# TAMUCrypto/virgo-plus

Hardware: AMD Instinct MI355X
Metric: prover sec + field-ops/sec, SHA-256 circuit, 1/2/4/8 MI355X (bit-exact) (higher is better)
Workload: dtype u64 (F_p^2, p=2^61-1); 1 GPU; SHA-256 1024-block circuit (SHA256_64.pws x1024, 102347776 gates, 15 layers, 2^23 input wires), GKR sumcheck + Virgo FFT/LDT commit on GPU (BASELINE configs[2]); pass_mode=sync, field_ops_per_proof=8299342697

## Files before the change

### virgo-plus_amd/__init__.py

```python
import ctypes
import os
import shutil
import subprocess

PKG_DIR = os.path.dirname(os.path.abspath(__file__))
ROOT = os.path.dirname(PKG_DIR)
CSRC = os.path.join(PKG_DIR, "csrc")
HOST = os.path.join(PKG_DIR, "host")
LIB_GPU = os.environ.get("VP_LIBGPU") or os.path.join(CSRC, "libvpgpu.so")
LIB_GPU_CHECKED = os.path.join(ROOT, "tools", "_build", "checked", "libvpgpu.so")
LIB_GPU_TESTDRV = os.path.join(ROOT, "tools", "_build", "testdrv", "libvpgpu.so")
LIB_HOST = os.path.join(HOST, "libvphost.so")
CLI = os.path.join(HOST, "virgo_plus_run")

GPU_SRC = [os.path.join(CSRC, f) for f in ("vpgpu.hip", "vpgpu_batched.inc", "vpgpu_pc.inc", "vpgpu_pc_shard.inc", "vpgpu_fftgkr.inc", "vpgpu_upload.inc", "vp_kernels_fftgkr.h", "vp_kernels.h", "vp_kernels_round.h", "vp_kernels_persist.h", "vp_kernels_batch.h",
                                              "vp_kernels_plan.h", "vp_kernels_pc.h", "vp_kernels_ntt8.h", "vp_kernels_ntt_long.h", "vp_keccak_asm.h", "vp_check.h", "vp_field.h")] + [
    os.path.join(ROOT, "include", "vpgpu.h")]
HOST_SRC = [os.path.join(HOST, f) for f in ("circuit.cpp", "prover.cpp", "verifier.cpp", "vphost.cpp")]
HOST_HDR = [os.path.join(HOST, f) for f in ("circuit.hpp", "prover.hpp", "verifier.hpp", "vphost.h", "field.hpp",
                                              "polynomial.hpp")]


def _stale(target, sources):
    if not os.path.exists(target):
        return True
    t = os.path.getmtime(target)
    return any(os.path.getmtime(s) > t for s in sources if os.path.exists(s))


def _hipcc():
    for c in (shutil.which("hipcc"), "/opt/rocm/bin/hipcc"):
        if c and os.path.exists(c):
            return c
    return None


def build(force=False, verbose=False):
    def run(cmd):
        if verbose:
            print(" ".join(cmd), flush=True)
        subprocess.run(cmd, check=True)

    if os.environ.get("VP_LIBGPU"):
        pass
    elif force or _stale(LIB_GPU, GPU_SRC):
        hipcc = _hipcc()
        if hipcc is None:
            if os.path.exists(LIB_GPU):
                return
# ... 951 lines not shown
```

### virgo-plus_amd/csrc/vp_field.h

```cpp
#pragma once
#include <stdint.h>

#if defined(__HIPCC__)
#define VP_HD __host__ __device__ __forceinline__
#else
#define VP_HD inline
#endif

namespace vp {

typedef unsigned long long u64;
typedef unsigned int u32;
typedef unsigned __int128 u128;

constexpr u64 P61 = 2305843009213693951ull;

struct alignas(16) F {
    u64 re, im;
};

VP_HD F f_make(u64 re, u64 im) { F r; r.re = re; r.im = im; return r; }
VP_HD F f_zero() { return f_make(0, 0); }
VP_HD F f_one() { return f_make(1, 0); }
VP_HD bool f_eq(const F &a, const F &b) { return a.re == b.re && a.im == b.im; }
// ... 110 lines not shown
}
template <bool WEAK = false, bool MS = false>
VP_HD F f_mad31_rb(const F &a, u64 y, const F &c) {
    const Sp31 ar = split31(a.re), ai = split31(a.im), b = split31(y);
    return f_make(dot1_31<WEAK, MS>(ar, b, c.re), dot1_31<WEAK, MS>(ai, b, c.im));
}
template <bool WEAK, bool MS = false>
VP_HD F f_mad31c_rb(const F &a, u64 y, const F &c) {
    const Sp31 ar = split31(a.re), ai = split31(a.im), b = split31(y);
    return f_make(dot1_31c<WEAK, MS>(ar, b, c.re), dot1_31c<WEAK, MS>(ai, b, c.im));
}
template <bool MS = false>
VP_HD u64 dot4_31cc(const Sp31 &x0, const Sp31 &y0, const Sp31 &x1, const Sp31 &y1, const Sp31 &x2, const Sp31 &y2, const Sp31 &x3, const Sp31 &y3) {
    const u64 L = (u64) x0.lo * y0.lo + (u64) x1.lo * y1.lo + (u64) x2.lo * y2.lo + (u64) x3.lo * y3.lo;
    const u64 C = (u64) x0.lo * y0.hi + (u64) x0.hi * y0.lo + (u64) x1.lo * y1.hi + (u64) x1.hi * y1.lo
                + (u64) x2.lo * y2.hi + (u64) x2.hi * y2.lo + (u64) x3.lo * y3.hi + (u64) x3.hi * y3.lo;
    const u64 H = (u64) x0.hi * y0.hi + (u64) x1.hi * y1.hi + (u64) x2.hi * y2.hi + (u64) x3.hi * y3.hi;
    u64 s = c31_add<MS>(C, (L & P61) + (L >> 61)) + (H << 1);
    s = (s & P61) + (s >> 61);
    return s >= P61 ? s - P61 : s;
}
template <bool MS = false>
VP_HD F f_dot2cc(const F &a, const F &b, const F &c, const F &d) {
#if defined(__HIP_DEVICE_COMPILE__) && !defined(VP_MUL128)
    const Sp31 ar = split31(a.re), ai = split31(a.im), nai = split31(P61 - a.im), br = split31(b.re), bi = split31(b.im);
    const Sp31 cr = split31(c.re), ci = split31(c.im), nci = split31(P61 - c.im), dr = split31(d.re), di = split31(d.im);
    return f_make(dot4_31cc<MS>(ar, br, nai, bi, cr, dr, nci, di), dot4_31cc<MS>(ar, bi, ai, br, cr, di, ci, dr));
#else
    return f_add(f_mul128(a, b), f_mul128(c, d));
#endif
}
VP_HD F f_lerp(const F &a, const F &b, const F &r) { return f_add(a, f_mul(r, f_sub(b, a))); }

}
```

### virgo-plus_amd/csrc/vp_kernels_batch.h

```cpp
#pragma once
#include "vp_kernels_round.h"

namespace vp {

struct Half { const F *bf; const F *bs; int h1; int pad; };
__device__ __forceinline__ F half_at(const Half &h, u32 i) {
    return f_mul(h.bf[i & ((1u << h.h1) - 1)], h.bs[i >> h.h1]);
}
__device__ __forceinline__ F half_mad(const Half &h, u32 i, const F &c) {
    return f_mad31c<false, VP_MADSHIFT != 0>(h.bf[i & ((1u << h.h1) - 1)], h.bs[i >> h.h1], c);
}

struct InitArgs2 {
    const u32 *rowptr; const u32 *e_g; const u32 *e_x; const uint16_t *e_tl;
    Half hg, hu;
    F *const *vals;
    const F *gc;
    const F *Vu;
    const F *assert_r;
    F *V, *M, *A;
    const uint8_t *s_layer; const u32 *s_idx;
    u32 n_rows;
    int vreal;
    const unsigned long long *const *valsr;
};
__device__ __forceinline__ F mul_val(const InitArgs2 &a, const F &y, const F &t) {
    return a.vreal ? f_mad31c_rb<false>(t, y.re, f_zero()) : f_mul(y, t);
}
__device__ __forceinline__ F val_at(const InitArgs2 &a, int l, u32 x) {
    return (a.vreal && a.valsr) ? f_make(a.valsr[l][x], 0) : a.vals[l][x];
}

template <int PHASE>
__device__ __forceinline__ void contrib2(const InitArgs2 &a, u32 e, F &m, F &ad, const F &vu) {
    const u32 g = a.e_g[e], x = a.e_x[e], tl = a.e_tl[e];
    const int ty = (tl >> 8) & 0x7f;
    F t = half_at(a.hg, g);
    if (tl & 0x8000) t = f_mul(t, *a.assert_r);
    if (PHASE == 1) {
        const int l = tl & 0xff;
        F ty_ = f_zero();
        if (l != 0xff && VP_CHK_LAYER(l, x)) ty_ = mul_val(a, val_at(a, l, x), t);
        switch (ty) {
            case T_ADD: ad = f_add(ad, ty_); m = f_add(m, t); break;
            case T_SUB: ad = f_sub(ad, ty_); m = f_add(m, t); break;
            case T_ANTISUB: ad = f_add(ad, ty_); m = f_sub(m, t); break;
            case T_MUL: m = f_add(m, ty_); break;
            case T_NAAB: ad = f_add(ad, ty_); m = f_sub(m, ty_); break;
            case T_ANTINAAB: m = f_add(m, f_sub(t, ty_)); break;
            case T_ADDC: ad = f_add(ad, f_mul(a.gc[g], t)); m = f_add(m, t); break;
            case T_MULC: m = f_add(m, f_mul(a.gc[g], t)); break;
            case T_COPY: m = f_add(m, t); break;
            case T_NOT: ad = f_add(ad, t); m = f_sub(m, t); break;
            case T_XOR: ad = f_add(ad, ty_); m = f_add(m, f_sub(t, f_dbl(ty_))); break;
            default: break;
        }
    } else {
        t = f_mul(t, half_at(a.hu, x));
        const F tv = f_mul(t, vu);
        switch (ty) {
            case T_ADD: m = f_add(m, t); ad = f_add(ad, tv); break;
            case T_SUB: m = f_sub(m, t); ad = f_add(ad, tv); break;
            case T_ANTISUB: m = f_add(m, t); ad = f_sub(ad, tv); break;
            case T_MUL: m = f_add(m, tv); break;
            case T_NAAB: m = f_add(m, f_sub(t, tv)); break;
            case T_ANTINAAB: m = f_sub(m, tv); ad = f_add(ad, tv); break;
            case T_XOR: ad = f_add(ad, tv); m = f_add(m, f_sub(t, f_dbl(tv))); break;
            case T_COPY: ad = f_add(ad, tv); break;
            case T_NOT: ad = f_add(ad, f_sub(t, tv)); break;
            case T_ADDC: ad = f_add(ad, f_mul(t, f_add(a.gc[g], vu))); break;
            case T_MULC: ad = f_add(ad, f_mul(tv, a.gc[g])); break;
            default: break;
        }
    }
}

struct P1Entry { u32 g, x, tl; };
struct P1Vals { F bf, bs, y; };
__device__ __forceinline__ P1Entry p1_load(const InitArgs2 &a, u32 e) { P1Entry c; c.g = a.e_g[e]; c.x = a.e_x[e]; c.tl = a.e_tl[e]; return c; }
__device__ __forceinline__ P1Vals p1_gather(const InitArgs2 &a, const P1Entry &c) {
    P1Vals v;
    v.bf = a.hg.bf[c.g & ((1u << a.hg.h1) - 1)]; v.bs = a.hg.bs[c.g >> a.hg.h1];
    const int l = c.tl & 0xff;
    v.y = (l != 0xff && VP_CHK_LAYER(l, c.x)) ? val_at(a, l, c.x) : f_zero();
    return v;
}
__device__ __forceinline__ void p1_apply(const InitArgs2 &a, const P1Entry &c, const P1Vals &v, F &m, F &ad) {
    const int ty = (c.tl >> 8) & 0x7f;
    F t = f_mul(v.bf, v.bs);
    if (c.tl & 0x8000) t = f_mul(t, *a.assert_r);
    F ty_ = f_zero();
    if ((c.tl & 0xff) != 0xff) ty_ = mul_val(a, v.y, t);
    switch (ty) {
        case T_ADD: ad = f_add(ad, ty_); m = f_add(m, t); break;
        case T_SUB: ad = f_sub(ad, ty_); m = f_add(m, t); break;
        case T_ANTISUB: ad = f_add(ad, ty_); m = f_sub(m, t); break;
        case T_MUL: m = f_add(m, ty_); break;
        case T_NAAB: ad = f_add(ad, ty_); m = f_sub(m, ty_); break;
        case T_ANTINAAB: m = f_add(m, f_sub(t, ty_)); break;
        case T_ADDC: ad = f_add(ad, f_mul(a.gc[c.g], t)); m = f_add(m, t); break;
        case T_MULC: m = f_add(m, f_mul(a.gc[c.g], t)); break;
        case T_COPY: m = f_add(m, t); break;
        case T_NOT: ad = f_add(ad, t); m = f_sub(m, t); break;
        case T_XOR: ad = f_add(ad, ty_); m = f_add(m, f_sub(t, f_dbl(ty_))); break;
        default: break;
    }
}

template <int PHASE>
__device__ __forceinline__ void init2_light_body(const InitArgs2 &a, u32 bid) {
    u32 row = bid * blockDim.x + threadIdx.x;
    if (row >= a.n_rows) return;
    if (PHASE == 2) {
        const int l = a.s_layer[row];
        if (l != 0xfe) a.V[row] = (l == 0xff || !VP_CHK((unsigned) l < g_vp_chk_layers() && a.s_idx[row] < g_vp_chk_lsize(l), 2, l, a.s_idx[row], row)) ? f_zero() : val_at(a, l, a.s_idx[row]);
    }
    u32 b = a.rowptr[row], e = a.rowptr[row + 1];
    if (!VP_CHK(b <= e, 3, row, b, e)) return;
    if (e - b > VP_LIGHT_MAX) return;
    F m = f_zero(), ad = f_zero();
    const F vu = PHASE == 2 ? *a.Vu : f_zero();
    for (u32 k = b; k < e; ++k) contrib2<PHASE>(a, k, m, ad, vu);
    a.M[row] = m;
    a.A[row] = ad;
}
template <int PHASE>
__global__ void __launch_bounds__(VP_BLOCK) k_init2_light(InitArgs2 a) { init2_light_body<PHASE>(a, blockIdx.x); }

struct ChunkFuse { const u32 *chunk_h; const u32 *heavy_row; const u32 *heavy_cptr; u32 *heavy_cnt; F *M; F *A; };
template <int PHASE>
__device__ __forceinline__ void init2_chunks_body(const InitArgs2 &a, const u32 *__restrict__ chunk_beg, const u32 *__restrict__ chunk_end,
                                                  u32 n_chunks, F *__restrict__ part, u32 bid, const ChunkFuse *fuse = nullptr) {
    const u32 c = bid * (blockDim.x >> 6) + (threadIdx.x >> 6);
    if (c >= n_chunks) return;
    const int lane = threadIdx.x & 63;
    F m = f_zero(), ad = f_zero();
    const F vu = PHASE == 2 ? *a.Vu : f_zero();
    for (u32 k = chunk_beg[c] + lane; k < chunk_end[c]; k += 64) contrib2<PHASE>(a, k, m, ad, vu);
    m = wave_sum(m);
    ad = wave_sum(ad);
    if (!fuse) { if (lane == 0) { part[2 * c] = m; part[2 * c + 1] = ad; } return; }
    const u32 h = fuse->chunk_h[c], c0 = fuse->heavy_cptr[h], n = fuse->heavy_cptr[h + 1] - c0, row = fuse->heavy_row[h];
    if (n == 1) { if (lane == 0) { fuse->M[row] = m; fuse->A[row] = ad; } return; }
    int last = 0;
    if (lane == 0) {
        unsigned long long *w = reinterpret_cast<unsigned long long *>(part + 2 * c);
        cf_st(w, m.re); cf_st(w + 1, m.im); cf_st(w + 2, ad.re); cf_st(w + 3, ad.im);
        asm volatile("s_waitcnt vmcnt(0)" ::: "memory");
        last = __hip_atomic_fetch_add(fuse->heavy_cnt + h, 1u, __ATOMIC_RELAXED, __HIP_MEMORY_SCOPE_AGENT) == n - 1;
    }
    last = __builtin_amdgcn_readfirstlane(last);
    if (!last) return;
    F tm = f_zero(), ta = f_zero();
    for (u32 i = lane; i < n; i += 64) {
        const unsigned long long *w = reinterpret_cast<const unsigned long long *>(part + 2 * (c0 + i));
        tm = f_add(tm, f_make(cf_ld(w), cf_ld(w + 1))); ta = f_add(ta, f_make(cf_ld(w + 2), cf_ld(w + 3)));
    }
    tm = wave_sum(tm); ta = wave_sum(ta);
    if (lane == 0) { fuse->M[row] = tm; fuse->A[row] = ta; __hip_atomic_store(fuse->heavy_cnt + h, 0u, __ATOMIC_RELAXED, __HIP_MEMORY_SCOPE_AGENT); }
}
template <int PHASE>
__global__ void __launch_bounds__(VP_BLOCK)
k_init2_chunks(InitArgs2 a, const u32 *__restrict__ chunk_beg, const u32 *__restrict__ chunk_end, u32 n_chunks,
               F *__restrict__ part) { init2_chunks_body<PHASE>(a, chunk_beg, chunk_end, n_chunks, part, blockIdx.x); }

__device__ __forceinline__ void liu_gather_body(const u32 *__restrict__ rowptr, const uint8_t *__restrict__ e_q, const u32 *__restrict__ e_g,
                                                const Half *__restrict__ H, u32 size, F *__restrict__ M, u32 bid, u32 u0 = 0) {
    u32 u = bid * blockDim.x + threadIdx.x;
    if (u >= size) return;
    F m = half_at(H[0], u0 + u);
    if (!VP_CHK(rowptr[u] <= rowptr[u + 1], 4, u, rowptr[u], rowptr[u + 1])) return;
    for (u32 k = rowptr[u]; k < rowptr[u + 1]; ++k) if (VP_CHK(e_q[k] < g_vp_chk_liu(), 4, u, k, e_q[k])) m = f_add(m, half_at(H[e_q[k]], e_g[k]));
    M[u] = m;
// ... 45 lines not shown
    const F dv = f_sub_lazy(v1, v0), dm = f_sub_lazy(m1, m0);
    lz_add(X, f_mad_lazy<true>(dm, dv, f_zero()));
    if (keep_y) lz_add(Y, f_mad_c<true>(m1, v1, HAS_A ? a1 : f_zero()));
    lz_add(Z, f_mad_c<true>(m0, v0, HAS_A ? a0 : f_zero()));
    vo = sf_fold<false>(r, dv, v0);
    mo = sf_fold<false>(r, dm, m0);
    if (HAS_A) ao = sf_fold<false>(r, f_sub_lazy(a1, a0), a0);
}

template <bool HAS_A>
__device__ __forceinline__ void sf_pair_step_rv(u64 v0, u64 v1, const F &m0, const F &m1, const F &a0, const F &a1,
                                                const F &r, Lz &X, Lz &Y, Lz &Z, F &vo, F &mo, F &ao, bool keep_y) {
    const u64 dv = v1 + P61 - v0;
    const F dm = f_sub_lazy(m1, m0);
    lz_add(X, f_mad31_rb<true, VP_MADSHIFT>(dm, dv, f_zero()));
    if (keep_y) lz_add(Y, f_mad31c_rb<true, VP_MADSHIFT>(m1, v1, HAS_A ? a1 : f_zero()));
    lz_add(Z, f_mad31c_rb<true, VP_MADSHIFT>(m0, v0, HAS_A ? a0 : f_zero()));
    vo = f_mad31c_rb<false, VP_MADSHIFT>(r, dv, f_make(v0, 0));
    mo = sf_fold<false>(r, dm, m0);
    if (HAS_A) ao = sf_fold<false>(r, f_sub_lazy(a1, a0), a0);
}

struct Sf3bLds { F s1[3][256]; F s2[3][128]; F red[4][9]; Lz acc2[3][128]; Lz acc3[3][64]; F dred[4]; };

struct GenLoad { static constexpr int MODE = 0; };
struct GenP1 {
    static constexpr int MODE = 1;
    const InitArgs2 *a; Half dot_h; F *dot_part;
    __device__ __forceinline__ void row(u32 row, u32 valid, F &m, F &ad) const {
        m = f_zero(); ad = f_zero();
        if (row >= valid || row >= a->n_rows) return;
        const u32 b = a->rowptr[row], e = a->rowptr[row + 1];
        if (e - b > VP_LIGHT_MAX) { m = a->M[row]; ad = a->A[row]; return; }
        for (u32 k = b; k < e; ++k) contrib2<1>(*a, k, m, ad, f_zero());
    }
    __device__ __forceinline__ void ptrs(u32 r0, u32 valid, u32 &b0, u32 &e0, u32 &e1) const {
        const u32 lim = min(valid, a->n_rows);
        b0 = e0 = e1 = 0;
        if (r0 >= lim) return;
        b0 = a->rowptr[r0]; e0 = a->rowptr[r0 + 1];
        e1 = r0 + 1 < lim ? a->rowptr[r0 + 2] : e0;
    }
    __device__ __forceinline__ void row2(u32 r0, u32 valid, u32 b0, u32 e0, u32 e1, F &m0, F &a0, F &m1, F &a1) const {
        m0 = f_zero(); a0 = f_zero(); m1 = f_zero(); a1 = f_zero();
        const u32 lim = min(valid, a->n_rows);
        if (r0 >= lim) return;
        const bool heavy0 = e0 - b0 > VP_LIGHT_MAX, heavy1 = e1 - e0 > VP_LIGHT_MAX;
        const bool f0 = !heavy0 && e0 > b0, f1 = !heavy1 && e1 > e0;
        P1Entry c0{}, c1{};
        if (f0) c0 = p1_load(*a, b0);
        if (f1) c1 = p1_load(*a, e0);
        P1Vals v0{}, v1{};
        if (f0) v0 = p1_gather(*a, c0);
        if (f1) v1 = p1_gather(*a, c1);
        if (heavy0) { m0 = a->M[r0]; a0 = a->A[r0]; }
        if (heavy1) { m1 = a->M[r0 + 1]; a1 = a->A[r0 + 1]; }
        if (f0) p1_apply(*a, c0, v0, m0, a0);
        if (f1) p1_apply(*a, c1, v1, m1, a1);
        if (!heavy0) for (u32 k = b0 + 1; k < e0; ++k) contrib2<1>(*a, k, m0, a0, f_zero());
        if (!heavy1) for (u32 k = e0 + 1; k < e1; ++k) contrib2<1>(*a, k, m1, a1, f_zero());
    }
};
struct GenLiu {
    static constexpr int MODE = 2;
    const u32 *rowptr; const uint8_t *e_q; const u32 *e_g; const Half *H;
    __device__ __forceinline__ void row(u32 u, u32 valid, F &m, F &ad) const {
        ad = f_zero(); m = f_zero();
        if (u >= valid) return;
        m = half_at(H[0], u);
        for (u32 k = rowptr[u]; k < rowptr[u + 1]; ++k) m = f_add(m, half_at(H[e_q[k]], e_g[k]));
    }
    __device__ __forceinline__ void ptrs(u32 u0, u32 valid, u32 &b0, u32 &e0, u32 &e1) const {
        b0 = e0 = e1 = 0;
        if (u0 >= valid) return;
        b0 = rowptr[u0]; e0 = rowptr[u0 + 1];
        e1 = u0 + 1 < valid ? rowptr[u0 + 2] : e0;
    }
    __device__ __forceinline__ void row2(u32 u0, u32 valid, u32 b0, u32 e0, u32 e1, F &m0, F &a0, F &m1, F &a1) const {
        m0 = f_zero(); a0 = f_zero(); m1 = f_zero(); a1 = f_zero();
        if (u0 >= valid) return;
        const bool ok1 = u0 + 1 < valid;
        const Half h0 = H[0];
        const F bf0 = h0.bf[u0 & ((1u << h0.h1) - 1)], bs0 = h0.bs[u0 >> h0.h1];
        F bf1 = f_zero(), bs1 = f_zero();
        if (ok1) { bf1 = h0.bf[(u0 + 1) & ((1u << h0.h1) - 1)]; bs1 = h0.bs[(u0 + 1) >> h0.h1]; }
        const bool f0 = e0 > b0, f1 = e1 > e0;
        u32 q0 = 0, g0 = 0, q1 = 0, g1 = 0;
        if (f0) { q0 = e_q[b0]; g0 = e_g[b0]; }
        if (f1) { q1 = e_q[e0]; g1 = e_g[e0]; }
        Half hq0 = h0, hq1 = h0;
        if (f0) hq0 = H[q0];
        if (f1) hq1 = H[q1];
        F xf0 = f_zero(), xs0 = f_zero(), xf1 = f_zero(), xs1 = f_zero();
        if (f0) { xf0 = hq0.bf[g0 & ((1u << hq0.h1) - 1)]; xs0 = hq0.bs[g0 >> hq0.h1]; }
        if (f1) { xf1 = hq1.bf[g1 & ((1u << hq1.h1) - 1)]; xs1 = hq1.bs[g1 >> hq1.h1]; }
        m0 = f_dot2cc<VP_MADSHIFT != 0>(bf0, bs0, xf0, xs0);
        if (ok1) m1 = f_dot2cc<VP_MADSHIFT != 0>(bf1, bs1, xf1, xs1);
        for (u32 k = b0 + 1; k < e0; ++k) m0 = half_mad(H[e_q[k]], e_g[k], m0);
        for (u32 k = e0 + 1; k < e1; ++k) m1 = half_mad(H[e_q[k]], e_g[k], m1);
    }
};

struct GenP2 {
    static constexpr int MODE = 3;
    const InitArgs2 *a;
    __device__ __forceinline__ F vrow(u32 row, u32 vend) const {
        if (row >= vend || row >= a->n_rows) return f_zero();
        const int l = a->s_layer[row];
        if (l == 0xff || l == 0xfe) return f_zero();
        const u32 x = a->s_idx[row];
        if (!VP_CHK((unsigned) l < g_vp_chk_layers() && x < g_vp_chk_lsize(l), 2, l, x, row)) return f_zero();
        return val_at(*a, l, x);
    }
    __device__ __forceinline__ void ptrs(u32 r0, u32 valid, u32 &b0, u32 &e0, u32 &e1) const {
        const u32 lim = min(valid, a->n_rows);
        b0 = e0 = e1 = 0;
        if (r0 >= lim) return;
        b0 = a->rowptr[r0]; e0 = a->rowptr[r0 + 1];
        e1 = r0 + 1 < lim ? a->rowptr[r0 + 2] : e0;
    }
    __device__ __forceinline__ void row2(u32 r0, u32 valid, u32 b0, u32 e0, u32 e1, F &m0, F &a0, F &m1, F &a1) const {
        m0 = f_zero(); a0 = f_zero(); m1 = f_zero(); a1 = f_zero();
        const u32 lim = min(valid, a->n_rows);
        if (r0 >= lim) return;
        const bool heavy0 = e0 - b0 > VP_LIGHT_MAX, heavy1 = e1 - e0 > VP_LIGHT_MAX;
        if (heavy0) { m0 = a->M[r0]; a0 = a->A[r0]; }
        if (heavy1) { m1 = a->M[r0 + 1]; a1 = a->A[r0 + 1]; }
        const F vu = *a->Vu;
        u32 k0 = heavy0 ? e0 : b0, k1 = heavy1 ? e1 : e0;
        while (k0 < e0 && k1 < e1) { contrib2<2>(*a, k0++, m0, a0, vu); contrib2<2>(*a, k1++, m1, a1, vu); }
        for (; k0 < e0; ++k0) contrib2<2>(*a, k0, m0, a0, vu);
        for (; k1 < e1; ++k1) contrib2<2>(*a, k1, m1, a1, vu);
    }
};

template <bool HAS_A, class Gen>
__device__ __forceinline__ void sumfold3b_body(const SfArgs &a, u32 bid, u32 nb, Sf3bLds &sm, const Gen &gen) {
    F (&s1)[3][256] = sm.s1; F (&s2)[3][128] = sm.s2; F (&red)[4][9] = sm.red;
    const int t = threadIdx.x, lane = t & 63, w = t >> 6;
    Lz acc[3];
#pragma unroll
    for (int i = 0; i < 3; ++i) acc[i].re = acc[i].im = 0;
    if (t < 128) { for (int i = 0; i < 3; ++i) { sm.acc2[i][t].re = 0; sm.acc2[i][t].im = 0; } }
    if (t < 64) { for (int i = 0; i < 3; ++i) { sm.acc3[i][t].re = 0; sm.acc3[i][t].im = 0; } }
    const F r0 = a.r[0], r1 = a.r[1], r2 = a.r[2];
    const bool keep_y0 = (a.keep_y0 & 1) != 0, keep_rest = (a.keep_y0 & 2) != 0;
    const bool vreal = (a.keep_y0 & 4) != 0;
    F dacc = f_zero();
    for (u32 c = bid; c < a.total_chunks; c += nb) {
        int j = 0;
        while (j + 1 < a.n_tab && c >= a.t[j + 1].chunk_start) ++j;
        const SfTab td = a.t[j];
        const u32 cl = c - td.chunk_start;
        const int wl = w, tl = t;
        const u32 i0 = td.off + cl * 512 + 2 * tl, vend = td.off + td.valid;
        {
            F v0, v1, m0, m1, a0 = f_zero(), a1 = f_zero();
            if constexpr (Gen::MODE == 3) { v0 = gen.vrow(i0, vend); v1 = gen.vrow(i0 + 1, vend); }
            else if (vreal && a.inVr) {
                v0 = f_make(i0 < vend ? a.inVr[i0] : 0ull, 0); v1 = f_make(i0 + 1 < vend ? a.inVr[i0 + 1] : 0ull, 0);
            } else {
                if (cl * 512 + 512 <= td.valid) { v0 = a.inV[i0]; v1 = a.inV[i0 + 1]; }
                else { v0 = ld_or_zero(a.inV, i0, vend); v1 = ld_or_zero(a.inV, i0 + 1, vend); }
            }
            if constexpr (Gen::MODE == 0) {
// ... 102 lines not shown
```

### virgo-plus_amd/csrc/vp_kernels_plan.h

```cpp
#pragma once
#include "vp_kernels_batch.h"

namespace vp {

#ifndef VP_SEG_LOG
#define VP_SEG_LOG 10
#endif
#define VP_SEG (1 << VP_SEG_LOG)
#define VP_SEG_THREADS 768

struct SegTab {
    u32 off;
    u32 valid;
    u32 seg_start;
    int seg_log;
};
struct SegArgs {
    const F *inV, *inM, *inA;
    F *outV, *outM, *outA;
    const F *r;
    F *part;
    u32 part_stride;
    u32 total_segs;
    int n_tab, n_rounds;
// ... 457 lines not shown
__global__ void __launch_bounds__(VP_BLOCK) k_dotfin_multi(const DotJob *__restrict__ jobs) {
    __shared__ F lds[4];
    const DotJob &j = jobs[blockIdx.x];
    F acc[1] = {f_zero()};
    for (u32 i = threadIdx.x; i < j.nblk; i += blockDim.x) acc[0] = f_add(acc[0], j.part[i]);
    block_sum<1>(acc, lds);
    if (threadIdx.x == 0) *j.out = acc[0];
}
__global__ void k_vu_place(const F *__restrict__ sums, F *const *__restrict__ dst, u32 n) {
    const u32 c = blockIdx.x * blockDim.x + threadIdx.x;
    if (c >= n) return;
    F v = sums[c];
    v.re = m_red128((u128) v.re); v.im = m_red128((u128) v.im);
    *dst[c] = v;
}
__global__ void __launch_bounds__(VP_BLOCK) k_chunks_multi(const ChunkJob *__restrict__ jobs, const BlkMap *__restrict__ map) {
    const BlkMap m = map[blockIdx.x];
    const ChunkJob &j = jobs[m.job];
    if (j.phase == 1) init2_chunks_body<1>(j.a, j.chunk_beg, j.chunk_end, j.n_chunks, j.part, m.bid, j.fused ? &j.fuse : nullptr);
    else init2_chunks_body<2>(j.a, j.chunk_beg, j.chunk_end, j.n_chunks, j.part, m.bid, j.fused ? &j.fuse : nullptr);
}
__global__ void __launch_bounds__(VP_BLOCK) k_combine_multi(const CombineJob *__restrict__ jobs, const BlkMap *__restrict__ map) {
    const BlkMap m = map[blockIdx.x];
    const CombineJob &j = jobs[m.job];
    init_combine_body(j.heavy_row, j.heavy_cptr, j.n_heavy, j.part, j.M, j.A, m.bid);
}
__global__ void __launch_bounds__(VP_BLOCK, VP_SF_MINB) k_sumfold3b_multi(const SfArgs *__restrict__ jobs, const BlkMap *__restrict__ map) {
    __shared__ Sf3bLds sm;
    const BlkMap m = map[blockIdx.x];
    const SfArgs &a = jobs[m.job];
    if (a.has_a) sumfold3b_body<true>(a, m.bid, a.nblk, sm, GenLoad()); else sumfold3b_body<false>(a, m.bid, a.nblk, sm, GenLoad());
}
struct SfGenJob { SfArgs sf; InitArgs2 a; GatherJob g; Half dot_h; F *dot_part; int mode; int pad; };
__global__ void __launch_bounds__(VP_BLOCK, VP_SF_MINB) k_sumfold3b_gen_multi(const SfGenJob *__restrict__ jobs, const BlkMap *__restrict__ map) {
    __shared__ Sf3bLds sm;
    const BlkMap m = map[blockIdx.x];
    const SfGenJob &j = jobs[m.job];
    if (j.mode == 1) {
        GenP1 g; g.a = &j.a; g.dot_h = j.dot_h; g.dot_part = j.dot_part;
        sumfold3b_body<true>(j.sf, m.bid, j.sf.nblk, sm, g);
    } else if (j.mode == 3) {
        GenP2 g; g.a = &j.a;
        sumfold3b_body<true>(j.sf, m.bid, j.sf.nblk, sm, g);
    } else {
        GenLiu g; g.rowptr = j.g.rowptr; g.e_q = j.g.e_q; g.e_g = j.g.e_g; g.H = j.g.H;
        sumfold3b_body<false>(j.sf, m.bid, j.sf.nblk, sm, g);
    }
}
__global__ void __launch_bounds__(VP_SEG_THREADS) k_seg_multi(const SegArgs *__restrict__ jobs, const BlkMap *__restrict__ map) {
    __shared__ SegLds sm;
    const BlkMap m = map[blockIdx.x];
    const SegArgs &a = jobs[m.job];
    if (a.has_a) seg_body<true>(a, m.bid, a.nblk, sm); else seg_body<false>(a, m.bid, a.nblk, sm);
}
__global__ void __launch_bounds__(VP_EMIT_THREADS) k_emit_multi(const EmitArgs *__restrict__ jobs) {
    extern __shared__ __align__(16) unsigned char smem_raw[];
    emit_body(jobs[blockIdx.x], smem_raw);
}

}
```

### virgo-plus_amd/csrc/vp_kernels_round.h

```cpp
#pragma once
#include <hip/hip_runtime.h>
#include "vp_field.h"

namespace vp {

#define VP_MAX_TAB 64
#define VP_BLOCK 256
#define VP_LIGHT_MAX 16
#define VP_CHUNK 512

enum { T_MUL = 0, T_ADD, T_SUB, T_ANTISUB, T_NAAB, T_ANTINAAB, T_INPUT, T_MULC, T_ADDC, T_XOR, T_NOT, T_COPY };

__device__ __forceinline__ F ldF(const F *p) { return *p; }

template <int CTRL, int ROW_MASK>
__device__ __forceinline__ u64 dpp_u64(u64 v) {
    const u32 lo = __builtin_amdgcn_update_dpp(0u, (u32) v, CTRL, ROW_MASK, 0xf, false);
    const u32 hi = __builtin_amdgcn_update_dpp(0u, (u32) (v >> 32), CTRL, ROW_MASK, 0xf, false);
    return ((u64) hi << 32) | lo;
}
__device__ __forceinline__ u64 m_fold(u64 s) {
    s = (s & P61) + (s >> 61);
    return s >= P61 ? s - P61 : s;
}
__device__ __forceinline__ F wave_sum63(F x) {
    u64 a = x.re, b = x.im;
    a += dpp_u64<0x111, 0xf>(a); b += dpp_u64<0x111, 0xf>(b);
    a += dpp_u64<0x112, 0xf>(a); b += dpp_u64<0x112, 0xf>(b);
    a += dpp_u64<0x114, 0xf>(a); b += dpp_u64<0x114, 0xf>(b);
    a = m_fold(a); b = m_fold(b);
    a += dpp_u64<0x118, 0xf>(a); b += dpp_u64<0x118, 0xf>(b);
    a += dpp_u64<0x142, 0xa>(a); b += dpp_u64<0x142, 0xa>(b);
    a += dpp_u64<0x143, 0xc>(a); b += dpp_u64<0x143, 0xc>(b);
    return f_make(m_fold(a), m_fold(b));
}
__device__ __forceinline__ F wave_sum(F x) {
    const F t = wave_sum63(x);
    F r;
    r.re = ((u64) __builtin_amdgcn_readlane((u32) (t.re >> 32), 63) << 32) | (u32) __builtin_amdgcn_readlane((u32) t.re, 63);
    r.im = ((u64) __builtin_amdgcn_readlane((u32) (t.im >> 32), 63) << 32) | (u32) __builtin_amdgcn_readlane((u32) t.im, 63);
    return r;
}

template <int N>
__device__ __forceinline__ void block_sum(F (&x)[N], F *lds ) {
    const int lane = threadIdx.x & 63, w = threadIdx.x >> 6;
#pragma unroll
    for (int i = 0; i < N; ++i) x[i] = wave_sum(x[i]);
    if (lane == 0) {
#pragma unroll
        for (int i = 0; i < N; ++i) lds[w * N + i] = x[i];
    }
    __syncthreads();
    if (threadIdx.x == 0) {
        const int nw = blockDim.x >> 6;
#pragma unroll
// ... 123 lines not shown
__global__ void __launch_bounds__(VP_BLOCK)
k_beta_expand(const F *__restrict__ bf, const F *__restrict__ bs, int h1, u32 count, F *__restrict__ out) {
    const u32 mask = (1u << h1) - 1;
    for (u32 i = blockIdx.x * blockDim.x + threadIdx.x; i < count; i += gridDim.x * blockDim.x)
        out[i] = f_mul(bf[i & mask], bs[i >> h1]);
}

__global__ void k_scale_entries(F *beta, const u32 *__restrict__ idx, u32 n, const F *__restrict__ s) {
    u32 i = blockIdx.x * blockDim.x + threadIdx.x;
    if (i < n) beta[idx[i]] = f_mul(beta[idx[i]], *s);
}

struct InitArgs {
    const u32 *rowptr;
    const u32 *e_g;
    const u32 *e_x;
    const uint16_t *e_tl;
    const F *beta_g;
    const F *beta_u;
    F *const *vals;
    const F *gc;
    const F *coef;
    F *M, *A;
    u32 n_rows;
};

template <int PHASE>
__device__ __forceinline__ void contrib(const InitArgs &a, u32 e, F &m, F &ad) {
    const u32 g = a.e_g[e];
    const u32 x = a.e_x[e];
    const u32 tl = a.e_tl[e];
    const int ty = (tl >> 8) & 0x7f;
    if (PHASE == 1) {
        const F t = a.beta_g[g];
        const int l = tl & 0xff;
        F ty_ = f_zero();
        if (l != 0xff) ty_ = f_mul(a.vals[l][x], t);
        switch (ty) {
            case T_ADD: ad = f_add(ad, ty_); m = f_add(m, t); break;
            case T_SUB: ad = f_sub(ad, ty_); m = f_add(m, t); break;
            case T_ANTISUB: ad = f_add(ad, ty_); m = f_sub(m, t); break;
            case T_MUL: m = f_add(m, ty_); break;
            case T_NAAB: ad = f_add(ad, ty_); m = f_sub(m, ty_); break;
            case T_ANTINAAB: m = f_add(m, f_sub(t, ty_)); break;
            case T_ADDC: ad = f_add(ad, f_mul(a.gc[g], t)); m = f_add(m, t); break;
            case T_MULC: m = f_add(m, f_mul(a.gc[g], t)); break;
            case T_COPY: m = f_add(m, t); break;
            case T_NOT: ad = f_add(ad, t); m = f_sub(m, t); break;
            case T_XOR: ad = f_add(ad, ty_); m = f_add(m, f_sub(t, f_dbl(ty_))); break;
            default: break;
        }
    } else {
        const F t = f_mul(a.beta_g[g], a.beta_u[x]);
        F cm = a.coef[2 * ty], ca = a.coef[2 * ty + 1];
        if (ty == T_ADDC) ca = f_add(a.gc[g], ca);
        if (ty == T_MULC) ca = f_mul(a.gc[g], ca);
        m = f_add(m, f_mul(t, cm));
        ad = f_add(ad, f_mul(t, ca));
    }
}

template <int PHASE>
__global__ void __launch_bounds__(VP_BLOCK) k_init_light(InitArgs a) {
    u32 row = blockIdx.x * blockDim.x + threadIdx.x;
    if (row >= a.n_rows) return;
    u32 b = a.rowptr[row], e = a.rowptr[row + 1];
    if (e - b > VP_LIGHT_MAX) return;
    F m = f_zero(), ad = f_zero();
    for (u32 k = b; k < e; ++k) contrib<PHASE>(a, k, m, ad);
    a.M[row] = m;
    a.A[row] = ad;
}

template <int PHASE>
__global__ void __launch_bounds__(VP_BLOCK)
k_init_chunks(InitArgs a, const u32 *__restrict__ chunk_beg, const u32 *__restrict__ chunk_end, u32 n_chunks,
              F *__restrict__ part) {
    const u32 c = blockIdx.x * (blockDim.x >> 6) + (threadIdx.x >> 6);
    if (c >= n_chunks) return;
    const int lane = threadIdx.x & 63;
    F m = f_zero(), ad = f_zero();
    for (u32 k = chunk_beg[c] + lane; k < chunk_end[c]; k += 64) contrib<PHASE>(a, k, m, ad);
    m = wave_sum(m);
    ad = wave_sum(ad);
// ... 53 lines not shown
}
__global__ void __launch_bounds__(VP_BLOCK)
k_liu_scatter(const F *__restrict__ bf, const F *__restrict__ bs, int h1, const u32 *__restrict__ dad, u32 n, F *M) {
    const u32 mask = (1u << h1) - 1;
    for (u32 g = blockIdx.x * blockDim.x + threadIdx.x; g < n; g += gridDim.x * blockDim.x) {
        const u32 u = dad[g];
        M[u] = f_add(M[u], f_mul(bf[g & mask], bs[g >> h1]));
    }
}

struct TabDesc {
    u32 off;
    u32 len_in;
    u32 valid_in;
    u32 pair_start;
};
struct RoundArgs {
    const F *inV, *inM, *inA;
    F *outV, *outM, *outA;
    const F *rp;
    F rv;
    int n_tab;
    int fold;
    int has_a;
    u32 total_pairs;
    unsigned long long skip;
    int add_off;
    TabDesc t[VP_MAX_TAB];
};

__device__ __forceinline__ F f_sub_lazy(const F &a, const F &b) { return f_make(a.re + P61 - b.re, a.im + P61 - b.im); }
template <bool WEAK = false> __device__ __forceinline__ F f_mad_lazy(const F &a, const F &b, const F &c) { return f_mad31<WEAK, VP_MADSHIFT>(a, b, c); }
template <bool WEAK = false> __device__ __forceinline__ F f_mad_c(const F &a, const F &b, const F &c) { return f_mad31c<WEAK, VP_MADSHIFT>(a, b, c); }
struct Lz { u64 re, im; };
__device__ __forceinline__ void lz_add(Lz &s, const F &x) { s.re += x.re; s.im += x.im; }
__device__ __forceinline__ void lz_fold(Lz &s) { s.re = (s.re & P61) + (s.re >> 61); s.im = (s.im & P61) + (s.im >> 61); }
__device__ __forceinline__ F lz_canon(const Lz &s) { return f_make(m_fold(s.re), m_fold(s.im)); }
__device__ __forceinline__ unsigned long long cf_ld(const unsigned long long *p) { return __hip_atomic_load(p, __ATOMIC_RELAXED, __HIP_MEMORY_SCOPE_AGENT); }
__device__ __forceinline__ void cf_st(unsigned long long *p, unsigned long long v) { __hip_atomic_store(p, v, __ATOMIC_RELAXED, __HIP_MEMORY_SCOPE_AGENT); }
__device__ __forceinline__ F ld_or_zero(const F *p, u32 i, u32 valid) { return i < valid ? p[i] : f_zero(); }

#define VP_BIG_PAIRS 32768
__device__ __forceinline__ F fold_entry(const F &e0, const F &e1, const F &r) { return f_mad_c(r, f_sub_lazy(e1, e0), e0); }
__device__ __forceinline__ void round_main_body(const RoundArgs &a, u32 bid, u32 nb, F (&acc)[3], F *lds) {
    const F r = a.rp ? *a.rp : a.rv;
    Lz X{0, 0}, Y{0, 0}, Z{0, 0};
    for (u32 q = bid * blockDim.x + threadIdx.x; q < a.total_pairs; q += nb * blockDim.x) {
        int j = 0;
        while (j + 1 < a.n_tab && q >= a.t[j + 1].pair_start) ++j;
        const TabDesc td = a.t[j];
        const u32 p = q - td.pair_start;
        F v0, v1, m0, m1, a0 = f_zero(), a1 = f_zero();
        if (a.fold) {
            const u32 i0 = td.off + 4 * p, vi = td.off + td.valid_in;
            const u32 vo = (td.valid_in + 1) >> 1;
            F e0 = ld_or_zero(a.inV, i0, vi), e1 = ld_or_zero(a.inV, i0 + 1, vi);
            F e2 = ld_or_zero(a.inV, i0 + 2, vi), e3 = ld_or_zero(a.inV, i0 + 3, vi);
            v0 = fold_entry(e0, e1, r); v1 = fold_entry(e2, e3, r);
            e0 = ld_or_zero(a.inM, i0, vi); e1 = ld_or_zero(a.inM, i0 + 1, vi);
            e2 = ld_or_zero(a.inM, i0 + 2, vi); e3 = ld_or_zero(a.inM, i0 + 3, vi);
            m0 = fold_entry(e0, e1, r); m1 = fold_entry(e2, e3, r);
            const u32 o0 = td.off + 2 * p;
            const bool w1 = 2 * p + 1 < vo;
            a.outV[o0] = v0; a.outM[o0] = m0;
            if (w1) { a.outV[o0 + 1] = v1; a.outM[o0 + 1] = m1; }
            if (a.has_a) {
                e0 = ld_or_zero(a.inA, i0, vi); e1 = ld_or_zero(a.inA, i0 + 1, vi);
                e2 = ld_or_zero(a.inA, i0 + 2, vi); e3 = ld_or_zero(a.inA, i0 + 3, vi);
                a0 = fold_entry(e0, e1, r); a1 = fold_entry(e2, e3, r);
                a.outA[o0] = a0;
// ... 198 lines not shown
```

Before: 165.0 billion field-ops/s.

## Replace per-gate switch with branchless table-driven lazy accumulation in init kernels

Gate contributions in the GKR init kernels move from a switch over gate types, with a full modular add/sub per term, to a branchless form. Compile-time coefficient masks select, negate and double each term, and the terms go into lazily reduced 64-bit accumulators that are canonicalised once at the end. Constant and assert multiplies are guarded by wave-wide ballots. The aim is to remove divergence between lanes handling different gate types and to cut per-gate reduction work, in exchange for always computing the operand products. The launch-bounds min-blocks for the sumfold gen kernel is also set to a fixed value of 4.

```diff
diff --git a/virgo-plus_amd/__init__.py b/virgo-plus_amd/__init__.py
--- a/virgo-plus_amd/__init__.py
+++ b/virgo-plus_amd/__init__.py
@@ -14,7 +14,7 @@
 CLI = os.path.join(HOST, "virgo_plus_run")
 
 GPU_SRC = [os.path.join(CSRC, f) for f in ("vpgpu.hip", "vpgpu_batched.inc", "vpgpu_pc.inc", "vpgpu_pc_shard.inc", "vpgpu_fftgkr.inc", "vpgpu_upload.inc", "vp_kernels_fftgkr.h", "vp_kernels.h", "vp_kernels_round.h", "vp_kernels_persist.h", "vp_kernels_batch.h",
-                                              "vp_kernels_plan.h", "vp_kernels_pc.h", "vp_kernels_ntt8.h", "vp_kernels_ntt_long.h", "vp_keccak_asm.h", "vp_check.h", "vp_field.h")] + [
+                                              "vp_kernels_plan.h", "vp_kernels_pc.h", "vp_kernels_ntt8.h", "vp_kernels_ntt_long.h", "vp_keccak_asm.h", "vp_check.h", "vp_field.h", "vp_gate.h")] + [
     os.path.join(ROOT, "include", "vpgpu.h")]
 HOST_SRC = [os.path.join(HOST, f) for f in ("circuit.cpp", "prover.cpp", "verifier.cpp", "vphost.cpp")]
 HOST_HDR = [os.path.join(HOST, f) for f in ("circuit.hpp", "prover.hpp", "verifier.hpp", "vphost.h", "field.hpp",
diff --git a/virgo-plus_amd/csrc/vp_field.h b/virgo-plus_amd/csrc/vp_field.h
--- a/virgo-plus_amd/csrc/vp_field.h
+++ b/virgo-plus_amd/csrc/vp_field.h
@@ -166,4 +166,13 @@
 }
 VP_HD F f_lerp(const F &a, const F &b, const F &r) { return f_add(a, f_mul(r, f_sub(b, a))); }
 
+VP_HD u64 m_fold(u64 s) {
+    s = (s & P61) + (s >> 61);
+    return s >= P61 ? s - P61 : s;
 }
+struct Lz { u64 re, im; };
+VP_HD void lz_add(Lz &s, const F &x) { s.re += x.re; s.im += x.im; }
+VP_HD void lz_fold(Lz &s) { s.re = (s.re & P61) + (s.re >> 61); s.im = (s.im & P61) + (s.im >> 61); }
+VP_HD F lz_canon(const Lz &s) { return f_make(m_fold(s.re), m_fold(s.im)); }
+
+}
diff --git a/virgo-plus_amd/csrc/vp_gate.h b/virgo-plus_amd/csrc/vp_gate.h
--- /dev/null
+++ b/virgo-plus_amd/csrc/vp_gate.h
@@ -0,0 +1,93 @@
+#pragma once
+#include "vp_field.h"
+
+namespace vp {
+
+enum { T_MUL = 0, T_ADD, T_SUB, T_ANTISUB, T_NAAB, T_ANTINAAB, T_INPUT, T_MULC, T_ADDC, T_XOR, T_NOT, T_COPY, T_COUNT };
+
+struct GateCoef { signed char mt, mw, at, aw; };
+constexpr GateCoef GATE_COEF[2][T_COUNT] = {
+    {
+         {0, 1, 0, 0},  {1, 0, 0, 1},  {1, 0, 0, -1},  {-1, 0, 0, 1},  {0, -1, 0, 1},  {1, -1, 0, 0},
+         {0, 0, 0, 0},  {0, 1, 0, 0},  {1, 0, 0, 1},  {1, -2, 0, 1},  {-1, 0, 1, 0},  {1, 0, 0, 0},
+    },
+    {
+         {0, 1, 0, 0},  {1, 0, 0, 1},  {-1, 0, 0, 1},  {1, 0, 0, -1},  {1, -1, 0, 0},  {0, -1, 0, 1},
+         {0, 0, 0, 0},  {0, 0, 0, 1},  {0, 0, 0, 1},  {1, -2, 0, 1},  {0, 0, 1, -1},  {0, 0, 0, 1},
+    },
+};
+constexpr int gate_coef(int phase, int ty, int which) {
+    return which == 0 ? GATE_COEF[phase - 1][ty].mt : which == 1 ? GATE_COEF[phase - 1][ty].mw : which == 2 ? GATE_COEF[phase - 1][ty].at : GATE_COEF[phase - 1][ty].aw;
+}
+constexpr u32 gate_mask(int phase, int which, int what) {
+    u32 m = 0;
+    for (int ty = 0; ty < T_COUNT; ++ty) {
+        const int c = gate_coef(phase, ty, which);
+        if (what == 0 ? c != 0 : what == 1 ? c < 0 : (c == 2 || c == -2)) m |= 1u << ty;
+    }
+    return m;
+}
+constexpr int gate_weight(int phase, int w0, int w1) {
+    int mx = 0;
+    for (int ty = 0; ty < T_COUNT; ++ty) {
+        const int a = gate_coef(phase, ty, w0), b = gate_coef(phase, ty, w1);
+        const int s = (a < 0 ? -a : a) + (b < 0 ? -b : b);
+        if (s > mx) mx = s;
+    }
+    return mx;
+}
+constexpr int GATE_WEIGHT_MAX = 3;
+static_assert(gate_weight(1, 0, 1) <= GATE_WEIGHT_MAX && gate_weight(1, 2, 3) <= GATE_WEIGHT_MAX &&
+              gate_weight(2, 0, 1) <= GATE_WEIGHT_MAX && gate_weight(2, 2, 3) <= GATE_WEIGHT_MAX, "gate_sum's overflow bound");
+constexpr u64 GATE_SUM_BOUND = P61 + 9 + GATE_WEIGHT_MAX * P61;
+static_assert((u128) (P61 + 9) + (u128) 2 * GATE_WEIGHT_MAX * P61 < ((u128) 1 << 64), "gate_sum's overflow bound");
+
+VP_HD u32 gate_bit(u32 tab, u32 ty) {
+#if defined(__HIP_DEVICE_COMPILE__)
+    return (u32) __builtin_amdgcn_sbfe((int) tab, ty, 1u);
+#else
+    return 0u - ((tab >> ty) & 1u);
+#endif
+}
+template <u32 NZ, u32 NEG, u32 DBL>
+VP_HD void gate_term(Lz &s, u32 ty, const F &x) {
+    if (NZ == 0) return;
+    u64 re = x.re, im = x.im;
+    if (NEG != 0) { const u32 n = gate_bit(NEG, ty); const u64 nn = ((u64) (n & (u32) (P61 >> 32)) << 32) | n; re ^= nn; im ^= nn; }
+    if (NZ != (1u << T_COUNT) - 1) { const u32 k = gate_bit(NZ, ty); const u64 kk = ((u64) k << 32) | k; re &= kk; im &= kk; }
+    const u32 d = DBL != 0 ? (DBL >> ty) & 1u : 0u;
+    s.re += re << d; s.im += im << d;
+}
+template <int PHASE>
+VP_HD void gate_sum(Lz &m, Lz &ad, u32 ty, const F &t, const F &w) {
+    lz_fold(m); lz_fold(ad);
+    gate_term<gate_mask(PHASE, 0, 0), gate_mask(PHASE, 0, 1), gate_mask(PHASE, 0, 2)>(m, ty, t);
+    gate_term<gate_mask(PHASE, 1, 0), gate_mask(PHASE, 1, 1), gate_mask(PHASE, 1, 2)>(m, ty, w);
+    gate_term<gate_mask(PHASE, 2, 0), gate_mask(PHASE, 2, 1), gate_mask(PHASE, 2, 2)>(ad, ty, t);
+    gate_term<gate_mask(PHASE, 3, 0), gate_mask(PHASE, 3, 1), gate_mask(PHASE, 3, 2)>(ad, ty, w);
+}
+
+VP_HD bool gate_any(bool c) {
+#if defined(__HIP_DEVICE_COMPILE__)
+    return __builtin_amdgcn_ballot_w64(c) != 0;
+#else
+    return c;
+#endif
+}
+
+template <int PHASE>
+VP_HD void gate_contrib(Lz &m, Lz &ad, u32 tl, F t, const F &h, const F &vu, const F *gc_g, const F *assert_r, bool vreal) {
+    const u32 ty = (tl >> 8) & 0xf;
+    const bool as = (tl & 0x8000) != 0;
+    if (gate_any(as)) { if (as) t = f_mul(t, *assert_r); }
+    F w;
+    if (PHASE == 1) w = vreal ? f_mad31c_rb<false>(t, h.re, f_zero()) : f_mul(h, t);
+    else { t = f_mul(t, h); w = f_mul(t, vu); }
+    const bool kc = ty == T_ADDC || ty == T_MULC;
+    if (gate_any(kc)) {
+        if (kc) w = PHASE == 1 ? f_mul(*gc_g, t) : ty == T_ADDC ? f_mul(t, f_add(*gc_g, vu)) : f_mul(w, *gc_g);
+    }
+    gate_sum<PHASE>(m, ad, ty, t, w);
+}
+
+}
diff --git a/virgo-plus_amd/csrc/vp_kernels_batch.h b/virgo-plus_amd/csrc/vp_kernels_batch.h
--- a/virgo-plus_amd/csrc/vp_kernels_batch.h
+++ b/virgo-plus_amd/csrc/vp_kernels_batch.h
@@ -24,55 +24,21 @@
     int vreal;
     const unsigned long long *const *valsr;
 };
-__device__ __forceinline__ F mul_val(const InitArgs2 &a, const F &y, const F &t) {
-    return a.vreal ? f_mad31c_rb<false>(t, y.re, f_zero()) : f_mul(y, t);
-}
 __device__ __forceinline__ F val_at(const InitArgs2 &a, int l, u32 x) {
     return (a.vreal && a.valsr) ? f_make(a.valsr[l][x], 0) : a.vals[l][x];
 }
 
+__device__ __forceinline__ F p1_operand(const InitArgs2 &a, u32 tl, u32 x) {
+    const int l = tl & 0xff;
+    const bool bin = l != 0xff && VP_CHK_LAYER(l, x);
+    return val_at(a, bin ? l : 0, bin ? x : 0u);
+}
 template <int PHASE>
-__device__ __forceinline__ void contrib2(const InitArgs2 &a, u32 e, F &m, F &ad, const F &vu) {
+__device__ __forceinline__ void contrib2(const InitArgs2 &a, u32 e, Lz &m, Lz &ad, const F &vu) {
     const u32 g = a.e_g[e], x = a.e_x[e], tl = a.e_tl[e];
-    const int ty = (tl >> 8) & 0x7f;
-    F t = half_at(a.hg, g);
-    if (tl & 0x8000) t = f_mul(t, *a.assert_r);
-    if (PHASE == 1) {
-        const int l = tl & 0xff;
-        F ty_ = f_zero();
-        if (l != 0xff && VP_CHK_LAYER(l, x)) ty_ = mul_val(a, val_at(a, l, x), t);
-        switch (ty) {
-            case T_ADD: ad = f_add(ad, ty_); m = f_add(m, t); break;
-            case T_SUB: ad = f_sub(ad, ty_); m = f_add(m, t); break;
-            case T_ANTISUB: ad = f_add(ad, ty_); m = f_sub(m, t); break;
-            case T_MUL: m = f_add(m, ty_); break;
-            case T_NAAB: ad = f_add(ad, ty_); m = f_sub(m, ty_); break;
-            case T_ANTINAAB: m = f_add(m, f_sub(t, ty_)); break;
-            case T_ADDC: ad = f_add(ad, f_mul(a.gc[g], t)); m = f_add(m, t); break;
-            case T_MULC: m = f_add(m, f_mul(a.gc[g], t)); break;
-            case T_COPY: m = f_add(m, t); break;
-            case T_NOT: ad = f_add(ad, t); m = f_sub(m, t); break;
-            case T_XOR: ad = f_add(ad, ty_); m = f_add(m, f_sub(t, f_dbl(ty_))); break;
-            default: break;
-        }
-    } else {
-        t = f_mul(t, half_at(a.hu, x));
-        const F tv = f_mul(t, vu);
-        switch (ty) {
-            case T_ADD: m = f_add(m, t); ad = f_add(ad, tv); break;
-            case T_SUB: m = f_sub(m, t); ad = f_add(ad, tv); break;
-            case T_ANTISUB: m = f_add(m, t); ad = f_sub(ad, tv); break;
-            case T_MUL: m = f_add(m, tv); break;
-            case T_NAAB: m = f_add(m, f_sub(t, tv)); break;
-            case T_ANTINAAB: m = f_sub(m, tv); ad = f_add(ad, tv); break;
-            case T_XOR: ad = f_add(ad, tv); m = f_add(m, f_sub(t, f_dbl(tv))); break;
-            case T_COPY: ad = f_add(ad, tv); break;
-            case T_NOT: ad = f_add(ad, f_sub(t, tv)); break;
-            case T_ADDC: ad = f_add(ad, f_mul(t, f_add(a.gc[g], vu))); break;
-            case T_MULC: ad = f_add(ad, f_mul(tv, a.gc[g])); break;
-            default: break;
-        }
-    }
+    const F t = half_at(a.hg, g);
+    const F h = PHASE == 1 ? p1_operand(a, tl, x) : half_at(a.hu, x);
+    gate_contrib<PHASE>(m, ad, tl, t, h, vu, a.gc + g, a.assert_r, a.vreal != 0);
 }
 
 struct P1Entry { u32 g, x, tl; };
@@ -81,30 +47,11 @@
 __device__ __forceinline__ P1Vals p1_gather(const InitArgs2 &a, const P1Entry &c) {
     P1Vals v;
     v.bf = a.hg.bf[c.g & ((1u << a.hg.h1) - 1)]; v.bs = a.hg.bs[c.g >> a.hg.h1];
-    const int l = c.tl & 0xff;
-    v.y = (l != 0xff && VP_CHK_LAYER(l, c.x)) ? val_at(a, l, c.x) : f_zero();
+    v.y = p1_operand(a, c.tl, c.x);
     return v;
 }
-__device__ __forceinline__ void p1_apply(const InitArgs2 &a, const P1Entry &c, const P1Vals &v, F &m, F &ad) {
-    const int ty = (c.tl >> 8) & 0x7f;
-    F t = f_mul(v.bf, v.bs);
-    if (c.tl & 0x8000) t = f_mul(t, *a.assert_r);
-    F ty_ = f_zero();
-    if ((c.tl & 0xff) != 0xff) ty_ = mul_val(a, v.y, t);
-    switch (ty) {
-        case T_ADD: ad = f_add(ad, ty_); m = f_add(m, t); break;
-        case T_SUB: ad = f_sub(ad, ty_); m = f_add(m, t); break;
-        case T_ANTISUB: ad = f_add(ad, ty_); m = f_sub(m, t); break;
-        case T_MUL: m = f_add(m, ty_); break;
-        case T_NAAB: ad = f_add(ad, ty_); m = f_sub(m, ty_); break;
-        case T_ANTINAAB: m = f_add(m, f_sub(t, ty_)); break;
-        case T_ADDC: ad = f_add(ad, f_mul(a.gc[c.g], t)); m = f_add(m, t); break;
-        case T_MULC: m = f_add(m, f_mul(a.gc[c.g], t)); break;
-        case T_COPY: m = f_add(m, t); break;
-        case T_NOT: ad = f_add(ad, t); m = f_sub(m, t); break;
-        case T_XOR: ad = f_add(ad, ty_); m = f_add(m, f_sub(t, f_dbl(ty_))); break;
-        default: break;
-    }
+__device__ __forceinline__ void p1_apply(const InitArgs2 &a, const P1Entry &c, const P1Vals &v, Lz &m, Lz &ad) {
+    gate_contrib<1>(m, ad, c.tl, f_mul(v.bf, v.bs), v.y, f_zero(), a.gc + c.g, a.assert_r, a.vreal != 0);
 }
 
 template <int PHASE>
@@ -118,11 +65,11 @@
     u32 b = a.rowptr[row], e = a.rowptr[row + 1];
     if (!VP_CHK(b <= e, 3, row, b, e)) return;
     if (e - b > VP_LIGHT_MAX) return;
-    F m = f_zero(), ad = f_zero();
+    Lz m{0, 0}, ad{0, 0};
     const F vu = PHASE == 2 ? *a.Vu : f_zero();
     for (u32 k = b; k < e; ++k) contrib2<PHASE>(a, k, m, ad, vu);
-    a.M[row] = m;
-    a.A[row] = ad;
+    a.M[row] = lz_canon(m);
+    a.A[row] = lz_canon(ad);
 }
 template <int PHASE>
 __global__ void __launch_bounds__(VP_BLOCK) k_init2_light(InitArgs2 a) { init2_light_body<PHASE>(a, blockIdx.x); }
@@ -134,11 +81,11 @@
     const u32 c = bid * (blockDim.x >> 6) + (threadIdx.x >> 6);
     if (c >= n_chunks) return;
     const int lane = threadIdx.x & 63;
-    F m = f_zero(), ad = f_zero();
+    Lz lm{0, 0}, la{0, 0};
     const F vu = PHASE == 2 ? *a.Vu : f_zero();
-    for (u32 k = chunk_beg[c] + lane; k < chunk_end[c]; k += 64) contrib2<PHASE>(a, k, m, ad, vu);
-    m = wave_sum(m);
-    ad = wave_sum(ad);
+    for (u32 k = chunk_beg[c] + lane; k < chunk_end[c]; k += 64) contrib2<PHASE>(a, k, lm, la, vu);
+    const F m = wave_sum(lz_canon(lm));
+    const F ad = wave_sum(lz_canon(la));
     if (!fuse) { if (lane == 0) { part[2 * c] = m; part[2 * c + 1] = ad; } return; }
     const u32 h = fuse->chunk_h[c], c0 = fuse->heavy_cptr[h], n = fuse->heavy_cptr[h + 1] - c0, row = fuse->heavy_row[h];
     if (n == 1) { if (lane == 0) { fuse->M[row] = m; fuse->A[row] = ad; } return; }
@@ -250,7 +197,9 @@
         if (row >= valid || row >= a->n_rows) return;
         const u32 b = a->rowptr[row], e = a->rowptr[row + 1];
         if (e - b > VP_LIGHT_MAX) { m = a->M[row]; ad = a->A[row]; return; }
-        for (u32 k = b; k < e; ++k) contrib2<1>(*a, k, m, ad, f_zero());
+        Lz lm{0, 0}, la{0, 0};
+        for (u32 k = b; k < e; ++k) contrib2<1>(*a, k, lm, la, f_zero());
+        m = lz_canon(lm); ad = lz_canon(la);
     }
     __device__ __forceinline__ void ptrs(u32 r0, u32 valid, u32 &b0, u32 &e0, u32 &e1) const {
         const u32 lim = min(valid, a->n_rows);
@@ -271,12 +220,14 @@
         P1Vals v0{}, v1{};
         if (f0) v0 = p1_gather(*a, c0);
         if (f1) v1 = p1_gather(*a, c1);
-        if (heavy0) { m0 = a->M[r0]; a0 = a->A[r0]; }
-        if (heavy1) { m1 = a->M[r0 + 1]; a1 = a->A[r0 + 1]; }
-        if (f0) p1_apply(*a, c0, v0, m0, a0);
-        if (f1) p1_apply(*a, c1, v1, m1, a1);
-        if (!heavy0) for (u32 k = b0 + 1; k < e0; ++k) contrib2<1>(*a, k, m0, a0, f_zero());
-        if (!heavy1) for (u32 k = e0 + 1; k < e1; ++k) contrib2<1>(*a, k, m1, a1, f_zero());
+        Lz lm0{0, 0}, la0{0, 0}, lm1{0, 0}, la1{0, 0};
+        if (heavy0) { const F m = a->M[r0], d = a->A[r0]; lm0 = Lz{m.re, m.im}; la0 = Lz{d.re, d.im}; }
+        if (heavy1) { const F m = a->M[r0 + 1], d = a->A[r0 + 1]; lm1 = Lz{m.re, m.im}; la1 = Lz{d.re, d.im}; }
+        if (f0) p1_apply(*a, c0, v0, lm0, la0);
+        if (f1) p1_apply(*a, c1, v1, lm1, la1);
+        if (!heavy0) for (u32 k = b0 + 1; k < e0; ++k) contrib2<1>(*a, k, lm0, la0, f_zero());
+        if (!heavy1) for (u32 k = e0 + 1; k < e1; ++k) contrib2<1>(*a, k, lm1, la1, f_zero());
+        m0 = lz_canon(lm0); a0 = lz_canon(la0); m1 = lz_canon(lm1); a1 = lz_canon(la1);
     }
 };
 struct GenLiu {
@@ -342,13 +293,15 @@
         const u32 lim = min(valid, a->n_rows);
         if (r0 >= lim) return;
         const bool heavy0 = e0 - b0 > VP_LIGHT_MAX, heavy1 = e1 - e0 > VP_LIGHT_MAX;
-        if (heavy0) { m0 = a->M[r0]; a0 = a->A[r0]; }
-        if (heavy1) { m1 = a->M[r0 + 1]; a1 = a->A[r0 + 1]; }
+        Lz lm0{0, 0}, la0{0, 0}, lm1{0, 0}, la1{0, 0};
+        if (heavy0) { const F m = a->M[r0], d = a->A[r0]; lm0 = Lz{m.re, m.im}; la0 = Lz{d.re, d.im}; }
+        if (heavy1) { const F m = a->M[r0 + 1], d = a->A[r0 + 1]; lm1 = Lz{m.re, m.im}; la1 = Lz{d.re, d.im}; }
         const F vu = *a->Vu;
         u32 k0 = heavy0 ? e0 : b0, k1 = heavy1 ? e1 : e0;
-        while (k0 < e0 && k1 < e1) { contrib2<2>(*a, k0++, m0, a0, vu); contrib2<2>(*a, k1++, m1, a1, vu); }
-        for (; k0 < e0; ++k0) contrib2<2>(*a, k0, m0, a0, vu);
-        for (; k1 < e1; ++k1) contrib2<2>(*a, k1, m1, a1, vu);
+        while (k0 < e0 && k1 < e1) { contrib2<2>(*a, k0++, lm0, la0, vu); contrib2<2>(*a, k1++, lm1, la1, vu); }
+        for (; k0 < e0; ++k0) contrib2<2>(*a, k0, lm0, la0, vu);
+        for (; k1 < e1; ++k1) contrib2<2>(*a, k1, lm1, la1, vu);
+        m0 = lz_canon(lm0); a0 = lz_canon(la0); m1 = lz_canon(lm1); a1 = lz_canon(la1);
     }
 };
 
diff --git a/virgo-plus_amd/csrc/vp_kernels_plan.h b/virgo-plus_amd/csrc/vp_kernels_plan.h
--- a/virgo-plus_amd/csrc/vp_kernels_plan.h
+++ b/virgo-plus_amd/csrc/vp_kernels_plan.h
@@ -513,7 +513,8 @@
     if (a.has_a) sumfold3b_body<true>(a, m.bid, a.nblk, sm, GenLoad()); else sumfold3b_body<false>(a, m.bid, a.nblk, sm, GenLoad());
 }
 struct SfGenJob { SfArgs sf; InitArgs2 a; GatherJob g; Half dot_h; F *dot_part; int mode; int pad; };
-__global__ void __launch_bounds__(VP_BLOCK, VP_SF_MINB) k_sumfold3b_gen_multi(const SfGenJob *__restrict__ jobs, const BlkMap *__restrict__ map) {
+#define VP_SFGEN_MINB 4
+__global__ void __launch_bounds__(VP_BLOCK, VP_SFGEN_MINB) k_sumfold3b_gen_multi(const SfGenJob *__restrict__ jobs, const BlkMap *__restrict__ map) {
     __shared__ Sf3bLds sm;
     const BlkMap m = map[blockIdx.x];
     const SfGenJob &j = jobs[m.job];
diff --git a/virgo-plus_amd/csrc/vp_kernels_round.h b/virgo-plus_amd/csrc/vp_kernels_round.h
--- a/virgo-plus_amd/csrc/vp_kernels_round.h
+++ b/virgo-plus_amd/csrc/vp_kernels_round.h
@@ -1,6 +1,7 @@
 #pragma once
 #include <hip/hip_runtime.h>
 #include "vp_field.h"
+#include "vp_gate.h"
 
 namespace vp {
 
@@ -8,8 +9,6 @@
 #define VP_BLOCK 256
 #define VP_LIGHT_MAX 16
 #define VP_CHUNK 512
-
-enum { T_MUL = 0, T_ADD, T_SUB, T_ANTISUB, T_NAAB, T_ANTINAAB, T_INPUT, T_MULC, T_ADDC, T_XOR, T_NOT, T_COPY };
 
 __device__ __forceinline__ F ldF(const F *p) { return *p; }
 
@@ -18,10 +17,6 @@
     const u32 lo = __builtin_amdgcn_update_dpp(0u, (u32) v, CTRL, ROW_MASK, 0xf, false);
     const u32 hi = __builtin_amdgcn_update_dpp(0u, (u32) (v >> 32), CTRL, ROW_MASK, 0xf, false);
     return ((u64) hi << 32) | lo;
-}
-__device__ __forceinline__ u64 m_fold(u64 s) {
-    s = (s & P61) + (s >> 61);
-    return s >= P61 ? s - P61 : s;
 }
 __device__ __forceinline__ F wave_sum63(F x) {
     u64 a = x.re, b = x.im;
@@ -211,24 +206,10 @@
     const u32 tl = a.e_tl[e];
     const int ty = (tl >> 8) & 0x7f;
     if (PHASE == 1) {
-        const F t = a.beta_g[g];
         const int l = tl & 0xff;
-        F ty_ = f_zero();
-        if (l != 0xff) ty_ = f_mul(a.vals[l][x], t);
-        switch (ty) {
-            case T_ADD: ad = f_add(ad, ty_); m = f_add(m, t); break;
-            case T_SUB: ad = f_sub(ad, ty_); m = f_add(m, t); break;
-            case T_ANTISUB: ad = f_add(ad, ty_); m = f_sub(m, t); break;
-            case T_MUL: m = f_add(m, ty_); break;
-            case T_NAAB: ad = f_add(ad, ty_); m = f_sub(m, ty_); break;
-            case T_ANTINAAB: m = f_add(m, f_sub(t, ty_)); break;
-            case T_ADDC: ad = f_add(ad, f_mul(a.gc[g], t)); m = f_add(m, t); break;
-            case T_MULC: m = f_add(m, f_mul(a.gc[g], t)); break;
-            case T_COPY: m = f_add(m, t); break;
-            case T_NOT: ad = f_add(ad, t); m = f_sub(m, t); break;
-            case T_XOR: ad = f_add(ad, ty_); m = f_add(m, f_sub(t, f_dbl(ty_))); break;
-            default: break;
-        }
+        Lz lm{m.re, m.im}, la{ad.re, ad.im};
+        gate_contrib<1>(lm, la, tl & 0x7fffu, a.beta_g[g], a.vals[l != 0xff ? l : 0][l != 0xff ? x : 0u], f_zero(), a.gc + g, nullptr, false);
+        m = lz_canon(lm); ad = lz_canon(la);
     } else {
         const F t = f_mul(a.beta_g[g], a.beta_u[x]);
         F cm = a.coef[2 * ty], ca = a.coef[2 * ty + 1];
@@ -348,10 +329,6 @@
 __device__ __forceinline__ F f_sub_lazy(const F &a, const F &b) { return f_make(a.re + P61 - b.re, a.im + P61 - b.im); }
 template <bool WEAK = false> __device__ __forceinline__ F f_mad_lazy(const F &a, const F &b, const F &c) { return f_mad31<WEAK, VP_MADSHIFT>(a, b, c); }
 template <bool WEAK = false> __device__ __forceinline__ F f_mad_c(const F &a, const F &b, const F &c) { return f_mad31c<WEAK, VP_MADSHIFT>(a, b, c); }
-struct Lz { u64 re, im; };
-__device__ __forceinline__ void lz_add(Lz &s, const F &x) { s.re += x.re; s.im += x.im; }
-__device__ __forceinline__ void lz_fold(Lz &s) { s.re = (s.re & P61) + (s.re >> 61); s.im = (s.im & P61) + (s.im >> 61); }
-__device__ __forceinline__ F lz_canon(const Lz &s) { return f_make(m_fold(s.re), m_fold(s.im)); }
 __device__ __forceinline__ unsigned long long cf_ld(const unsigned long long *p) { return __hip_atomic_load(p, __ATOMIC_RELAXED, __HIP_MEMORY_SCOPE_AGENT); }
 __device__ __forceinline__ void cf_st(unsigned long long *p, unsigned long long v) { __hip_atomic_store(p, v, __ATOMIC_RELAXED, __HIP_MEMORY_SCOPE_AGENT); }
 __device__ __forceinline__ F ld_or_zero(const F *p, u32 i, u32 valid) { return i < valid ? p[i] : f_zero(); }
```

Measured after the change: 162.4 billion field-ops/s. 0.984x the previous value.
